# c0gent/hbbft

Hardware: AMD Instinct MI355X
Metric: verified BLS sig shares/sec (whole node) + combine latency, N=64 f=21 (higher is better)
Workload: dtype u32 limbs (Fp, 14x28-bit); 1 GPU; ThresholdSign share verification, BASELINE configs[1]; batch_per_gpu=65536, streams=2, documents_per_gpu=1024, n_nodes=64, f=21, pairing_impl=auto, parallelism=shard-by-batch x1

## Files before the change

hbbft_amd/csrc/ofp.hpp:

```cpp
#pragma once
#include "qfp.hpp"

namespace hbs {

HP_D int o_idx() { return (int)((threadIdx.x >> 1) & 3); }

HP_D int32_t o_swz4(int32_t v) { return __builtin_amdgcn_ds_swizzle(v, 0x101F); }
HP_D Fp o_swz4_fp(const Fp& a) {
  Fp r;
#pragma unroll
  for (int i = 0; i < NL; i++) r.l[i] = o_swz4(a.l[i]);
  return r;
}

HP_D Fp o_sel(int o, const Fp& a0, const Fp& a1, const Fp& a2, const Fp& a3) {
  const bool b0 = (o & 1) != 0, b1 = (o & 2) != 0;
  Fp r;
#pragma unroll
  for (int i = 0; i < NL; i++) {
    const int32_t lo = b0 ? a1.l[i] : a0.l[i];
    const int32_t hi = b0 ? a3.l[i] : a2.l[i];
    r.l[i] = b1 ? hi : lo;
  }
  return r;
// ... 128 lines not shown
  o.c1.c2 = fp_mul(f.c1.c2, fp_const(hb::FROB2_5_C0));
  return o;
}

HP_D HLine h_dbl_step_o(HJac& T) {
  Fp r[4];
  {
    const Fp x[4] = {T.x, T.y, T.z, fp_add(T.y, T.z)};
    h_sqr4(x, r);
  }
  const Fp A = r[0], B = r[1], ZZ = r[2], YZ = r[3];
  const Fp E = fp_lin(3, A, 0, A);
  {
    const Fp xb = fp_add(T.x, B);
    const Fp x[4] = {B, xb, E, E}, y[4] = {B, xb, E, T.x};
    h_mul4(x, y, r);
  }
  const Fp C = r[0], XB = r[1], F = r[2], EX = r[3];
  const Fp D = fp_lin(2, fp_sub(fp_sub(XB, A), C), 0, C);
  const Fp Z3 = fp_sub(fp_sub(YZ, B), ZZ);
  const Fp X3 = fp_sub(F, fp_add(D, D));
  {
    const Fp x[4] = {E, Z3, E, E}, y[4] = {ZZ, ZZ, fp_sub(D, X3), ZZ};
    h_mul4(x, y, r);
  }
  HLine l;
  l.c0 = fp_reduce(fp_sub(EX, fp_add(B, B)));
  l.c1 = fp_neg(r[0]);
  l.c4 = r[1];
  T.y = fp_reduce(fp_sub(r[2], fp_lin(8, C, 0, C)));
  T.x = fp_reduce(X3);
  T.z = fp_reduce(Z3);
  return l;
}

HP_D HLine h_add_step_o(HJac& T, const Fp& xQ, const Fp& yQ) {
  Fp r[4];
  {
    const Fp x[4] = {T.z, yQ, T.z, T.z}, y[4] = {T.z, T.z, T.z, T.z};
    h_mul4(x, y, r);
  }
  const Fp Z1Z1 = r[0], YZ = r[1];
  {
    const Fp x[4] = {xQ, YZ, xQ, xQ}, y[4] = {Z1Z1, Z1Z1, Z1Z1, Z1Z1};
    h_mul4(x, y, r);
  }
  const Fp H = fp_sub(r[0], T.x);
  const Fp rr = fp_sub(r[1], T.y);
  {
    const Fp x[4] = {H, rr, T.z, H}, y[4] = {H, rr, H, H};
    h_mul4(x, y, r);
  }
  const Fp HH = r[0], R2 = r[1], Z3 = r[2];
  {
    const Fp x[4] = {H, T.x, yQ, rr}, y[4] = {HH, HH, Z3, xQ};
    h_mul4(x, y, r);
  }
  const Fp HHH = r[0], V = r[1], YZ3 = r[2], RX = r[3];
  const Fp X3 = fp_sub(fp_sub(R2, HHH), fp_add(V, V));
  {
    const Fp x[4] = {rr, T.y, rr, rr}, y[4] = {fp_sub(V, X3), HHH, fp_sub(V, X3), fp_sub(V, X3)};
    h_mul4(x, y, r);
  }
  HLine l;
  l.c0 = fp_reduce(fp_sub(RX, YZ3));
  l.c1 = fp_neg(rr);
  l.c4 = Z3;
  T.x = fp_reduce(X3);
  T.y = fp_reduce(fp_sub(r[0], r[1]));
  T.z = Z3;
  return l;
}

struct LaneOcto {
  static constexpr int LANES = 8;
  static HP_D bool leader() { return (threadIdx.x & 7) == 0; }
  static HP_D bool value_writer() { return o_idx() == 0; }
  using Walk = HJac;
  template <bool W1, bool W2, int GEN>
  using Park = NoPark;
  static HP_D HLine dbl_step(HJac& T) { return h_dbl_step_o(T); }
  static HP_D HLine add_step(HJac& T, const Fp& xQ, const Fp& yQ) { return h_add_step_o(T, xQ, yQ); }

  static HP_D H6 mul6(const H6& a, const H6& b) { return h6_mul_o(a, b); }
  template <class A1, class B1>
  static HP_D void mul6x2(const H6& a0, const H6& b0, const A1& a1, const B1& b1, H6& r0, H6& r1) {
    h6_mul_pair_o(a0, b0, h6_of(a1), h6_of(b1), r0, r1);
  }
  static HP_D void mul6x2_12(const H6& a0, const H6& b0, const H6& a1, const Fp& c1, const Fp& c2, H6& r0, H6& r1) {
    h6_mul_pair_o(a0, b0, a1, {h_zero(), c1, c2}, r0, r1);
  }
  static HP_D void line_product(const Fp& a0, const Fp& a1, const Fp& a4, const Fp& b0, const Fp& b1, const Fp& b4,
                                H6& C0, Fp& c11, Fp& c12) {
    Fp r[4];
    {
      const Fp x[4] = {a0, a1, a4, fp_addl(a0, a4)}, y[4] = {b0, b1, b4, fp_add(b0, b4)};
      h_mul4(x, y, r);
    }
    const Fp a0b0 = r[0], a1b1 = r[1], a4b4 = r[2], t04 = r[3];
    {
      const Fp x[4] = {fp_addl(a1, a4), fp_addl(a0, a1), a0, a0}, y[4] = {fp_add(b1, b4), fp_add(b0, b1), b0, b0};
      h_mul4(x, y, r);
    }
    h_line_comb(a0b0, a1b1, a4b4, t04, r[0], r[1], C0, c11, c12);
  }
  static HP_D H12 cyclo_sqr(const H12& f) { return h12_cyclo_sqr_o(f); }
  static HP_D H12 frob1(const H12& f) { return h12_frob1_o(f); }
  static HP_D H12 frob2(const H12& f) { return h12_frob2_o(f); }

  template <bool G1, bool G2, bool WALK_FIRST, class RA, class RB, class ST>
  static HP_D void lines_at_p(const RA& raw_a, const RB& raw_b, const ST& A, const ST& B, bool neg2, HLine& la,
                              HLine& lb, const NoPark&) {
    const HLine ra = raw_a();
    const HLine rb = raw_b();
    Fp r[4];
    const Fp x[4] = {ra.c1, ra.c4, rb.c1, rb.c4};
    const Fp y[4] = {side_xP<G1>(A), side_yP<G1>(A, false), side_xP<G2>(B), side_yP<G2>(B, neg2)};
    fp_mul4(x, y, r);
    la.c0 = A.act ? ra.c0 : h_one();
    la.c1 = A.act ? r[0] : fp_zero();
    la.c4 = A.act ? r[1] : fp_zero();
    lb.c0 = B.act ? rb.c0 : h_one();
    lb.c1 = B.act ? r[2] : fp_zero();
    lb.c4 = B.act ? r[3] : fp_zero();
  }
};

}
```

hbbft_amd/csrc/pair_side.hpp:

```cpp
#pragma once
#include "launch.hpp"
#include "qfp.hpp"

namespace hbs {

constexpr int PAIR_STEPS = 68;
constexpr int PL_Q4 = 11;
constexpr int STASH_WORDS = 72;
static_assert(PARK_WORDS <= STASH_WORDS, "the Miller loop parks T and P in the stash (pfp.hpp PairPark)");

HP_D void stash_fp(uint32_t* __restrict__ s, const Fp& a) {
  const Fp r = fp_reduce(a);
  Fp rp = fp_addl(r, fp_const(P_L));
  fp_norm(rp);
  const Fp c = (r.l[NL - 1] < 0) ? rp : r;
#pragma unroll
  for (int w = 0; w < 12; w++) {
    const int bit = 32 * w, li = bit / 28, sh = bit % 28;
    uint64_t v = (uint64_t)(uint32_t)c.l[li] >> sh;
    if (li + 1 < NL) v |= (uint64_t)(uint32_t)c.l[li + 1] << (28 - sh);
    if (li + 2 < NL) v |= (uint64_t)(uint32_t)c.l[li + 2] << (56 - sh);
    s[w * 256] = (uint32_t)v;
  }
}
// ... 113 lines not shown

template <class G, bool WALK, bool DBL, int SIDE, class ST, class PK>
HP_D HLine side_raw(const PairSide& s, ST& st, int step, const PK& pk) {
  if constexpr (!WALK) {
    return line_load(s.lines + line_at(st.q * PAIR_STEPS + step));
  } else if constexpr (DBL) {
    return pk.template walk<SIDE>(st, [&](typename G::Walk& T) HP_L { return G::dbl_step(T); });
  } else {
    Fp xQ, yQ;
    side_q(s, st, xQ, yQ);
    return pk.template walk<SIDE>(st, [&](typename G::Walk& T) HP_L { return G::add_step(T, xQ, yQ); });
  }
}

struct PairArgs {
  int n;
  PairSide s1, s2;
  int flags;
  uint8_t* verdict;
  uint32_t* value_out;
};


template <class G, bool PLUS1>
HP_D H12 exp_abs_x_gs(const H12& base) {
  const uint64_t e = PLUS1 ? hb::X_ABS + 1 : hb::X_ABS;
  H12 r = base;
#pragma unroll 1
  for (int k = 62; k >= 0; k--) {
    r = G::cyclo_sqr(r);
    if ((e >> k) & 1) r = h12_mul<G>(r, base);
  }
  return r;
}
template <class G>
struct ExpGs {
  HP_D H12 x(const H12& f) { return h12_conj(exp_abs_x_gs<G, false>(f)); }
  HP_D H12 xm1(const H12& f) { return h12_conj(exp_abs_x_gs<G, true>(f)); }
};

template <class G, class Exp>
HP_D H12 final_exp(const H12& f, uint32_t* __restrict__ stash) {
  const H12 f1 = h12_mul<G>(h12_conj(f), h12_inv<G>(f));
  const H12 g = h12_mul<G>(G::frob2(f1), f1);
  stash12(stash, g);
  Exp ex;
  H12 a = ex.xm1(ex.xm1(g));
  const H12 b = h12_mul<G>(ex.x(a), G::frob1(a));
  {
    const H12 gs = unstash12(stash);
    const H12 w = h12_mul<G>(h12_mul<G>(G::frob2(b), h12_conj(b)), h12_mul<G>(G::cyclo_sqr(gs), gs));
    stash12(stash, w);
  }
  const H12 c = ex.x(ex.x(b));
  return h12_mul<G>(c, unstash12(stash));
}

template <class G, class Exp, bool W1, bool W2, int GEN>
HP_D void lane_verify(const PairArgs& a, uint32_t* stash) {
  const int i = (int)((blockIdx.x * 256u + threadIdx.x) / (unsigned)G::LANES);
  if (i >= a.n) return;
  constexpr bool G1 = GEN == 1, G2 = GEN == 2;
  const bool neg2 = (a.flags & 1) != 0;
  SideStateT<typename G::Walk> A, B;
  const bool ok1 = side_init<W1, G1>(a.s1, i, false, A);
  const bool ok2 = side_init<W2, G2>(a.s2, i, neg2, B);
  if (!ok1 || !ok2) {
    if (G::leader() && a.verdict) a.verdict[i] = 0;
    return;
  }
  const typename G::template Park<W1, W2, GEN> pk(stash + threadIdx.x);
  pk.init(A, B);
  constexpr bool WF = !W1 && W2;
  H12 f = h12_one();
  int step = 0;
#pragma unroll 1
  for (int b = 62; b >= 0; b--) {
    if (b != 62) f = h12_sqr<G>(f);
    {
      HLine la, lb;
      G::template lines_at_p<G1, G2, WF>([&]() HP_L { return side_raw<G, W1, true, 0>(a.s1, A, step, pk); },
                                         [&]() HP_L { return side_raw<G, W2, true, 1>(a.s2, B, step, pk); }, A, B, neg2,
                                         la, lb, pk);
      f = h12_mul_lines<G>(f, la.c0, la.c1, la.c4, lb.c0, lb.c1, lb.c4);
    }
    step++;
    if ((hb::X_ABS >> b) & 1) {
      HLine la, lb;
      G::template lines_at_p<G1, G2, WF>([&]() HP_L { return side_raw<G, W1, false, 0>(a.s1, A, step, pk); },
                                         [&]() HP_L { return side_raw<G, W2, false, 1>(a.s2, B, step, pk); }, A, B, neg2,
                                         la, lb, pk);
      f = h12_mul_lines<G>(f, la.c0, la.c1, la.c4, lb.c0, lb.c1, lb.c4);
      step++;
    }
  }
  if (a.flags & 2) f = h12_conj(f);
  const H12 e = final_exp<G, Exp>(f, stash + threadIdx.x);
  if (a.value_out && G::value_writer()) {
    uint32_t* o = a.value_out + (size_t)i * 144 + (lp_even() ? 0 : 12);
    fp_to_words(e.c0.c0, o + 0);
    fp_to_words(e.c0.c1, o + 24);
    fp_to_words(e.c0.c2, o + 48);
    fp_to_words(e.c1.c0, o + 72);
    fp_to_words(e.c1.c1, o + 96);
    fp_to_words(e.c1.c2, o + 120);
  }
  const bool one = h12_is_one(e);
  if (G::leader() && a.verdict) a.verdict[i] = one ? 1 : 0;
}

}

namespace hbl {

inline hbs::PairArgs pair_args(int n, const PairSideDesc& d1, const PairSideDesc& d2, int flags, uint8_t* verdict,
                               uint32_t* value_out) {
  hbs::PairArgs a;
  a.n = n;
  const PairSideDesc* d[2] = {&d1, &d2};
  hbs::PairSide* o[2] = {&a.s1, &a.s2};
  for (int k = 0; k < 2; k++) {
    o[k]->p = (const uint32_t*)d[k]->p;
    o[k]->q = (const uint32_t*)d[k]->q;
    o[k]->lines = (const int4*)d[k]->lines;
    o[k]->qinf = d[k]->qinf;
    o[k]->idx = d[k]->idx;
    o[k]->nq = (uint32_t)d[k]->nq;
  }
  a.flags = flags;
  a.verdict = verdict;
  a.value_out = value_out;
  return a;
}

inline int pair_gen_mode(const PairSideDesc& d1, const PairSideDesc& d2) {
  return (d1.p == nullptr) == (d2.p == nullptr) ? 0 : (d1.p == nullptr ? 1 : 2);
}

template <class K, int GEN>
hipError_t lane_launch(hipStream_t s, int n, const PairSideDesc& d1, const PairSideDesc& d2, int flags,
                       uint8_t* verdict, uint32_t* value_out) {
  const hbs::PairArgs a = pair_args(n, d1, d2, flags, verdict, value_out);
  const dim3 grid((unsigned)((K::LANES * (size_t)n + 255) / 256)), block(256);
  const size_t lds = (size_t)hbs::STASH_WORDS * 256 * 4;
  const bool w1 = d1.lines == nullptr, w2 = d2.lines == nullptr;
  if (w1 && w2)
    hipLaunchKernelGGL((K::template kernel<true, true, GEN>), grid, block, lds, s, a);
  else if (w1)
    hipLaunchKernelGGL((K::template kernel<true, false, GEN>), grid, block, lds, s, a);
  else if (w2)
    hipLaunchKernelGGL((K::template kernel<false, true, GEN>), grid, block, lds, s, a);
  else
    hipLaunchKernelGGL((K::template kernel<false, false, GEN>), grid, block, lds, s, a);
  return hipGetLastError();
}

}
```

hbbft_amd/csrc/pfp.hpp:

```cpp
#pragma once
#include "sfp.hpp"
#include "words.hpp"

#ifndef HP_INV_MODE
#define HP_INV_MODE 0
#endif

#define HP_D __device__ __forceinline__
#define HP_L __attribute__((always_inline))

namespace hbs {

constexpr int DPP_SWAP = 0xB1;
constexpr int DPP_EVEN = 0xA0;
constexpr int DPP_ODD = 0xF5;

HP_D bool lp_even() { return (threadIdx.x & 1) == 0; }
template <int CTRL>
HP_D int32_t dpp(int32_t v) {
  return __builtin_amdgcn_mov_dpp(v, CTRL, 0xF, 0xF, true);
}
template <int CTRL>
HP_D Fp dpp_fp(const Fp& a) {
  Fp r;
// ... 133 lines not shown
#pragma unroll
      for (int i = 0; i <= N; i++) row[i] = (t[i] >> 31) | (t[i + 1] << 1);
      const uint32_t fl = hb::words_abs<N + 1>(row);
      ks ^= fl;
      ss ^= (uint32_t)dpp<DPP_SWAP>((int32_t)fl);
#pragma unroll
      for (int i = 0; i < N; i++) {
        mine[i] = row[i];
        other[i] = (uint32_t)dpp<DPP_SWAP>((int32_t)row[i]);
      }
    }
    {
      uint32_t t[N + 2], w[N + 2];
      hb::words_mul_sm<N, true>(co, sm, ss, t);
#pragma unroll
      for (int i = 0; i < N + 2; i++) t[i] = (uint32_t)dpp<DPP_SWAP>((int32_t)t[i]);
      const uint32_t xe = 0u - (co[N] >> 31);
      const uint32_t k0 = km & ks;
      const uint64_t q = (uint64_t)(((k0 + (co[0] ^ ks) * km + t[0]) * minv) & 0x7fffffffu);
      uint64_t c = k0;
#pragma unroll
      for (int i = 0; i < N + 2; i++) {
        const uint32_t xi = (i <= N ? co[i] : xe) ^ ks;
        c += (uint64_t)xi * km;
        if (i < N) c += q * mod[i];
        c += t[i];
        w[i] = (uint32_t)c;
        c >>= 32;
      }
#pragma unroll
      for (int i = 0; i <= N; i++) co[i] = (w[i] >> 31) | (w[i + 1] << 1);
    }
  }
  const uint32_t mine_one = hb::words_is_one<N>(mine) ? 1u : 0u;
  const uint32_t part_one = (uint32_t)dpp<DPP_SWAP>((int32_t)mine_one);
  const bool one = (ev ? part_one : mine_one) != 0;
  uint32_t v[N + 1];
#pragma unroll
  for (int i = 0; i <= N; i++) {
    const uint32_t pv = (uint32_t)dpp<DPP_SWAP>((int32_t)co[i]);
    v[i] = ev ? pv : co[i];
  }
  hb::words_reduce_32m<N>(v, mod);
#pragma unroll
  for (int i = 0; i < N; i++) out[i] = one ? v[i] : 0u;
}

template <int MODE = 0>
HP_D Fp h_inv_vartime(const Fp& a) {
  const Fp s = fp_sqr(a);
  const Fp n = fp_add(s, dpp_fp<DPP_SWAP>(s));
  uint32_t w[12], p[12], r[12];
  fp_to_words(n, w);
  uint32_t nz = 0;
#pragma unroll
  for (int i = 0; i < 12; i++) nz |= w[i];
  if (nz == 0) return fp_zero();
#pragma unroll
  for (int i = 0; i < 12; i++) p[i] = hb::PM2_W[i];
  p[0] += 2;
  if ((MODE & INV_PAIR) != 0)
    lp_inv_uniform<12>(w, p, r);
  else
    hb::words_inv_vartime<12, MODE>(w, p, r);
  return h_conj(fp_mul(a, fp_from_words(r)));
}

template <int M, int K>
HP_D Fp fp_red_mk(const Fp& t, const Fp& a) {
  const int64_t top = (int64_t)t.l[NL - 1] * M + (int64_t)K * a.l[NL - 1];
  const int32_t q = (int32_t)((top * QINV) >> 32);
  Fp r;
  int64_t acc = 0;
#pragma unroll
  for (int i = 0; i < NL - 1; i++) {
    acc += (int64_t)t.l[i] * M + (int64_t)K * a.l[i] - (int64_t)q * (int32_t)P_L[i];
    r.l[i] = (int32_t)acc & MASK28;
    acc >>= 28;
  }
  r.l[NL - 1] = (int32_t)(acc + top - (int64_t)q * (int32_t)P_L[NL - 1]);
  return r;
}
HP_D Fp fp_red_l(const Fp& t) { return fp_red_mk<1, 0>(t, t); }
HP_D Fp h_add_xi_l(const Fp& s, const Fp& t) {
  const int32_t sm = lp_even() ? -1 : 0;
  const Fp pt = dpp_fp<DPP_SWAP>(t);
  Fp r;
#pragma unroll
  for (int i = 0; i < NL; i++) r.l[i] = s.l[i] + t.l[i] + ((pt.l[i] ^ sm) - sm);
  return r;
}
HP_D Fp fp_sub2l(const Fp& a, const Fp& b, const Fp& c) {
  Fp r;
#pragma unroll
  for (int i = 0; i < NL; i++) r.l[i] = a.l[i] - b.l[i] - c.l[i];
  return r;
}

HP_D Fp h_xi_l(const Fp& t) {
  const int32_t sm = lp_even() ? -1 : 0;
  const Fp pt = dpp_fp<DPP_SWAP>(t);
  Fp r;
#pragma unroll
  for (int i = 0; i < NL; i++) r.l[i] = t.l[i] + ((pt.l[i] ^ sm) - sm);
  return r;
}

struct H6 { Fp c0, c1, c2; };
struct H12 { H6 c0, c1; };

HP_D H6 h6_zero() { return {h_zero(), h_zero(), h_zero()}; }
HP_D H6 h6_one() { return {h_one(), h_zero(), h_zero()}; }
HP_D H6 h6_add(const H6& a, const H6& b) { return {fp_add(a.c0, b.c0), fp_add(a.c1, b.c1), fp_add(a.c2, b.c2)}; }
HP_D H6 h6_sub(const H6& a, const H6& b) { return {fp_sub(a.c0, b.c0), fp_sub(a.c1, b.c1), fp_sub(a.c2, b.c2)}; }
HP_D H6 h6_neg(const H6& a) { return {fp_neg(a.c0), fp_neg(a.c1), fp_neg(a.c2)}; }
HP_D H6 h6_red(const H6& a) { return {fp_reduce(a.c0), fp_reduce(a.c1), fp_reduce(a.c2)}; }
HP_D H6 h6_mul_v(const H6& a) { return {h_mul_xi(a.c2), a.c0, a.c1}; }

HP_D H6 h6_mul(const H6& a, const H6& b) {
  const Fp v1 = h_mul(a.c1, b.c1);
  const Fp v2 = h_mul(a.c2, b.c2);
  const Fp d0 = fp_sub2l(h_mul(fp_addl(a.c1, a.c2), fp_add(b.c1, b.c2)), v1, v2);
  const Fp v0 = h_mul(a.c0, b.c0);
  const Fp c0 = fp_red_l(h_add_xi_l(v0, d0));
  const Fp c1 = fp_red_l(h_add_xi_l(fp_sub2l(h_mul(fp_addl(a.c0, a.c1), fp_add(b.c0, b.c1)), v0, v1), v2));
  const Fp c2 = fp_red_l(fp_addl(fp_sub2l(h_mul(fp_addl(a.c0, a.c2), fp_add(b.c0, b.c2)), v0, v2), v1));
  return {c0, c1, c2};
}
HP_D H6 h6_inv(const H6& a) {
  const Fp c0 = fp_reduce(fp_sub(h_sqr(a.c0), h_mul_xi(h_mul(a.c1, a.c2))));
  const Fp c1 = fp_reduce(fp_sub(h_mul_xi(h_sqr(a.c2)), h_mul(a.c0, a.c1)));
  const Fp c2 = fp_reduce(fp_sub(h_sqr(a.c1), h_mul(a.c0, a.c2)));
  const Fp t = fp_reduce(fp_add(h_mul(a.c0, c0), h_mul_xi(fp_add(h_mul(a.c2, c1), h_mul(a.c1, c2)))));
  const Fp ti = fp_reduce(h_inv_vartime<HP_INV_MODE>(t));
  return {h_mul(c0, ti), h_mul(c1, ti), h_mul(c2, ti)};
}

HP_D H12 h12_one() { return {h6_one(), h6_zero()}; }
HP_D H12 h12_conj(const H12& a) { return {a.c0, h6_neg(a.c1)}; }
HP_D H12 h12_red(const H12& a) { return {h6_red(a.c0), h6_red(a.c1)}; }
HP_D H12 h12_kcomb(const H6& t0, const H6& t1, const H6& s) {
  return {{fp_red_l(h_add_xi_l(t0.c0, t1.c2)), fp_red_l(fp_addl(t0.c1, t1.c0)), fp_red_l(fp_addl(t0.c2, t1.c1))},
          {fp_red_l(fp_sub2l(s.c0, t0.c0, t1.c0)), fp_red_l(fp_sub2l(s.c1, t0.c1, t1.c1)),
           fp_red_l(fp_sub2l(s.c2, t0.c2, t1.c2))}};
}

HP_D H6 h6_mul_12(const H6& x, const Fp& b1, const Fp& b2) {
  const Fp u = h_mul(x.c1, b1);
  const Fp w = h_mul(x.c2, b2);
  const Fp c0 = fp_red_l(h_xi_l(fp_sub2l(h_mul(fp_addl(x.c1, x.c2), fp_add(b1, b2)), u, w)));
  const Fp c1 = fp_red_l(h_add_xi_l(h_mul(x.c0, b1), w));
  const Fp c2 = fp_red_l(fp_addl(h_mul(x.c0, b2), u));
  return {c0, c1, c2};
}

HP_D const H6& h6_of(const H6& a) { return a; }
template <class F>
HP_D auto h6_of(const F& f) -> decltype(f()) { return f(); }

template <class G>
HP_D H12 h12_mul(const H12& a, const H12& b) {
  H6 t0, t1;
  G::mul6x2(a.c0, b.c0, a.c1, b.c1, t0, t1);
  const H6 s = G::mul6(h6_add(a.c0, a.c1), h6_add(b.c0, b.c1));
  return h12_kcomb(t0, t1, s);
}
template <class G>
HP_D H12 h12_sqr(const H12& a) {
  H6 t, s;
  G::mul6x2(a.c0, a.c1, [&]() HP_L { return h6_add(a.c0, a.c1); },
            [&]() HP_L { return h6_red(h6_add(a.c0, h6_mul_v(a.c1))); }, t, s);
  return {{fp_red_l(h_add_xi_l(fp_subl(s.c0, t.c0), fp_subl(fp_zero(), t.c2))), fp_red_l(fp_sub2l(s.c1, t.c1, t.c0)),
           fp_red_l(fp_sub2l(s.c2, t.c2, t.c1))},
          {fp_red_l(fp_addl(t.c0, t.c0)), fp_red_l(fp_addl(t.c1, t.c1)), fp_red_l(fp_addl(t.c2, t.c2))}};
}
template <class G>
HP_D H12 h12_mul_lines(const H12& f, const Fp& a0, const Fp& a1, const Fp& a4, const Fp& b0, const Fp& b1,
                       const Fp& b4) {
  H6 C0, t0, t1;
  Fp c11, c12;
  G::line_product(a0, a1, a4, b0, b1, b4, C0, c11, c12);
  G::mul6x2_12(f.c0, C0, f.c1, c11, c12, t0, t1);
  const H6 s = G::mul6(h6_add(f.c0, f.c1), {C0.c0, fp_add(C0.c1, c11), fp_add(C0.c2, c12)});
  return h12_kcomb(t0, t1, s);
}
template <class G>
HP_D H12 h12_inv(const H12& a) {
  H6 s0, s1, r0, r1;
  G::mul6x2(a.c0, a.c0, a.c1, a.c1, s0, s1);
  const H6 t = h6_red(h6_sub(h6_red(s0), h6_red(h6_mul_v(h6_red(s1)))));
  const H6 ti = h6_red(h6_inv(t));
  G::mul6x2(a.c0, ti, a.c1, ti, r0, r1);
  return h12_red({r0, h6_neg(r1)});
}

#define HP_FROB1(K) h_const(hb::FROB1_##K##_C0, hb::FROB1_##K##_C1)
HP_D H12 h12_frob1(const H12& f) {
  H12 r;
  r.c0.c0 = h_conj(f.c0.c0);
  r.c1.c0 = h_mul(h_conj(f.c1.c0), HP_FROB1(1));
  r.c0.c1 = h_mul(h_conj(f.c0.c1), HP_FROB1(2));
  r.c1.c1 = h_mul(h_conj(f.c1.c1), HP_FROB1(3));
  r.c0.c2 = h_mul(h_conj(f.c0.c2), HP_FROB1(4));
  r.c1.c2 = h_mul(h_conj(f.c1.c2), HP_FROB1(5));
  return h12_red(r);
}
HP_D H12 h12_frob2(const H12& f) {
  H12 r;
  r.c0.c0 = f.c0.c0;
  r.c1.c0 = fp_mul(f.c1.c0, fp_const(hb::FROB2_1_C0));
  r.c0.c1 = fp_mul(f.c0.c1, fp_const(hb::FROB2_2_C0));
  r.c1.c1 = fp_mul(f.c1.c1, fp_const(hb::FROB2_3_C0));
  r.c0.c2 = fp_mul(f.c0.c2, fp_const(hb::FROB2_4_C0));
  r.c1.c2 = fp_mul(f.c1.c2, fp_const(hb::FROB2_5_C0));
  return r;
}

HP_D H12 h12_cyclo_sqr(const H12& f) {
  const Fp& a0 = f.c0.c0; const Fp& a2 = f.c0.c1; const Fp& a4 = f.c0.c2;
  const Fp& a1 = f.c1.c0; const Fp& a3 = f.c1.c1; const Fp& a5 = f.c1.c2;
  H12 r;
  {
    const Fp s0 = h_sqr(a0), s3 = h_sqr(a3), s03 = h_sqr(fp_add(a0, a3));
    r.c0.c0 = fp_red_mk<3, -2>(h_add_xi_l(s0, s3), a0);
    r.c1.c1 = fp_red_mk<3, 2>(fp_sub2l(s03, s0, s3), a3);
  }
  {
    const Fp s1 = h_sqr(a1), s4 = h_sqr(a4), s14 = h_sqr(fp_add(a1, a4));
    r.c0.c1 = fp_red_mk<3, -2>(h_add_xi_l(s1, s4), a2);
    r.c1.c2 = fp_red_mk<3, 2>(fp_sub2l(s14, s1, s4), a5);
  }
  {
    const Fp s2 = h_sqr(a2), s5 = h_sqr(a5), s25 = h_sqr(fp_add(a2, a5));
    r.c0.c2 = fp_red_mk<3, -2>(h_add_xi_l(s2, s5), a4);
    r.c1.c0 = fp_red_mk<3, 2>(h_add_xi_l(fp_zero(), fp_sub2l(s25, s2, s5)), a1);
  }
  return r;
}

struct HC { Fp a1, a2, a4, a5; };

HP_D HC hc_compress(const H12& f) { return {f.c1.c0, f.c0.c1, f.c0.c2, f.c1.c2}; }
HP_D HC hc_sqr(const HC& c) {
  HC r;
  {
    const Fp s1 = h_sqr(c.a1), s4 = h_sqr(c.a4), s14 = h_sqr(fp_add(c.a1, c.a4));
    r.a2 = fp_red_mk<3, -2>(h_add_xi_l(s1, s4), c.a2);
    r.a5 = fp_red_mk<3, 2>(fp_sub2l(s14, s1, s4), c.a5);
  }
  {
    const Fp s2 = h_sqr(c.a2), s5 = h_sqr(c.a5), s25 = h_sqr(fp_add(c.a2, c.a5));
    r.a4 = fp_red_mk<3, -2>(h_add_xi_l(s2, s5), c.a4);
    r.a1 = fp_red_mk<3, 2>(h_add_xi_l(fp_zero(), fp_sub2l(s25, s2, s5)), c.a1);
  }
  return r;
}
HP_D Fp hc_denom(const Fp& a1) { return fp_lin(4, a1, 0, a1); }
HP_D H12 hc_decompress(const HC& c, const Fp& di) {
  const Fp s5 = h_sqr(c.a5), s2 = h_sqr(c.a2);
  Fp t = h_xi_l(s5);
#pragma unroll
  for (int i = 0; i < NL; i++) t.l[i] += 3 * s2.l[i];
  const Fp a3 = h_mul(fp_red_mk<1, -2>(t, c.a4), di);
  const Fp u = fp_addl(fp_lin(2, h_sqr(a3), -3, h_mul(c.a4, c.a2)), h_mul(c.a1, c.a5));
  const Fp a0 = fp_red_l(h_add_xi_l(h_one(), u));
  return {{a0, c.a2, c.a4}, {c.a1, a3, c.a5}};
}
// ... 82 lines not shown

constexpr int PARK_WORDS = 72;
constexpr int park_fit(int used, bool need, int words) { return need && used + words <= PARK_WORDS ? used : -1; }
typedef volatile __attribute__((address_space(3))) uint32_t* ParkCol;

HP_D void park_put(ParkCol c, int slot, const Fp& a) {
#pragma unroll
  for (int i = 0; i < NL; i++) c[(slot + i) * 256] = (uint32_t)a.l[i];
}
HP_D Fp park_get(ParkCol c, int slot) {
  Fp r;
#pragma unroll
  for (int i = 0; i < NL; i++) r.l[i] = (int32_t)c[(slot + i) * 256];
  return r;
}

template <bool W1, bool W2, int GEN>
struct PairPark {
  static constexpr int TW = 3 * NL, PW = 2 * NL;
  static constexpr int T_B = park_fit(0, W2, TW);
  static constexpr int U1 = T_B < 0 ? 0 : TW;
  static constexpr int T_A = park_fit(U1, W1, TW);
  static constexpr int U2 = U1 + (T_A < 0 ? 0 : TW);
  static constexpr int P_A = park_fit(U2, GEN != 1, PW);
  static constexpr int U3 = U2 + (P_A < 0 ? 0 : PW);
  static constexpr int P_B = park_fit(U3, GEN != 2, PW);
  template <int SIDE>
  static constexpr int t_slot() { return SIDE == 0 ? T_A : T_B; }
  template <int SIDE>
  static constexpr int p_slot() { return SIDE == 0 ? P_A : P_B; }

  ParkCol col;
  HP_D explicit PairPark(uint32_t* c) : col((ParkCol)c) {}

  template <int SIDE>
  HP_D void put_T(const HProj& T) const {
    park_put(col, t_slot<SIDE>(), T.x);
    park_put(col, t_slot<SIDE>() + NL, T.y);
    park_put(col, t_slot<SIDE>() + 2 * NL, T.z);
  }
  template <int SIDE, class ST>
  HP_D void init_side(const ST& st) const {
    if constexpr (t_slot<SIDE>() >= 0) put_T<SIDE>(st.T);
    if constexpr (p_slot<SIDE>() >= 0) {
      park_put(col, p_slot<SIDE>(), st.xP);
      park_put(col, p_slot<SIDE>() + NL, st.yP);
    }
  }
  template <class ST>
  HP_D void init(const ST& A, const ST& B) const {
    init_side<0>(A);
    init_side<1>(B);
  }
  template <int SIDE, class ST, class F>
  HP_D HLine walk(ST& st, const F& f) const {
    if constexpr (t_slot<SIDE>() < 0) {
      return f(st.T);
    } else {
      HProj T;
      T.z = park_get(col, t_slot<SIDE>() + 2 * NL);
      T.y = park_get(col, t_slot<SIDE>() + NL);
      T.x = park_get(col, t_slot<SIDE>());
      const HLine l = f(T);
      put_T<SIDE>(T);
      return l;
    }
  }
  template <int SIDE, class ST>
  HP_D Fp xP(const ST& st) const {
    if constexpr (p_slot<SIDE>() < 0) return st.xP; else return park_get(col, p_slot<SIDE>());
  }
  template <int SIDE, class ST>
  HP_D Fp yP(const ST& st) const {
    if constexpr (p_slot<SIDE>() < 0) return st.yP; else return park_get(col, p_slot<SIDE>() + NL);
  }
};

#ifndef HP_PARK
#define HP_PARK 1
#endif
#ifndef HP_WALK_FIRST
#define HP_WALK_FIRST 1
#endif

struct LanePair {
  static constexpr int LANES = 2;
  static HP_D bool leader() { return lp_even(); }
  static HP_D bool value_writer() { return true; }
  using Walk = HProj;
  static HP_D HLine dbl_step(HProj& T) { return h_dbl_step_h(T); }
  static HP_D HLine add_step(HProj& T, const Fp& xQ, const Fp& yQ) { return h_add_step_h(T, xQ, yQ); }

  static HP_D H6 mul6(const H6& a, const H6& b) { return h6_mul(a, b); }
  template <class A1, class B1>
  static HP_D void mul6x2(const H6& a0, const H6& b0, const A1& a1, const B1& b1, H6& r0, H6& r1) {
    r0 = h6_mul(a0, b0);
    r1 = h6_mul(h6_of(a1), h6_of(b1));
  }
  static HP_D void mul6x2_12(const H6& a0, const H6& b0, const H6& a1, const Fp& c1, const Fp& c2, H6& r0, H6& r1) {
    r0 = h6_mul(a0, b0);
    r1 = h6_mul_12(a1, c1, c2);
  }
  static HP_D void line_product(const Fp& a0, const Fp& a1, const Fp& a4, const Fp& b0, const Fp& b1, const Fp& b4,
                                H6& C0, Fp& c11, Fp& c12) {
    const Fp a0b0 = h_mul(a0, b0);
    const Fp a1b1 = h_mul(a1, b1);
    const Fp a4b4 = h_mul(a4, b4);
    c11 = fp_red_l(fp_sub2l(h_mul(fp_addl(a0, a4), fp_add(b0, b4)), a0b0, a4b4));
    c12 = fp_red_l(fp_sub2l(h_mul(fp_addl(a1, a4), fp_add(b1, b4)), a1b1, a4b4));
    C0 = {fp_red_l(h_add_xi_l(a0b0, a4b4)), fp_red_l(fp_sub2l(h_mul(fp_addl(a0, a1), fp_add(b0, b1)), a0b0, a1b1)),
          a1b1};
  }
  static HP_D H12 cyclo_sqr(const H12& f) { return h12_cyclo_sqr(f); }
  static HP_D H12 frob1(const H12& f) { return h12_frob1(f); }
  static HP_D H12 frob2(const H12& f) { return h12_frob2(f); }

#if HP_PARK
  template <bool W1, bool W2, int GEN>
  using Park = PairPark<W1, W2, GEN>;
#else
  template <bool W1, bool W2, int GEN>
  using Park = NoPark;
#endif

  template <bool GEN, int SIDE, class ST, class PK>
  static HP_D HLine line_at_p(const HLine& l, const ST& st, bool negate, const PK& pk) {
    HLine e;
    e.c0 = st.act ? l.c0 : h_one();
    const Fp c1 = fp_mul(l.c1, GEN ? side_xP<true>(st) : pk.template xP<SIDE>(st));
    e.c1 = st.act ? c1 : fp_zero();
    const Fp c4 = fp_mul(l.c4, GEN ? side_yP<true>(st, negate) : pk.template yP<SIDE>(st));
    e.c4 = st.act ? c4 : fp_zero();
    return e;
  }
  template <bool G1, bool G2, bool WALK_FIRST, class RA, class RB, class ST, class PK>
  static HP_D void lines_at_p(const RA& raw_a, const RB& raw_b, const ST& A, const ST& B, bool neg2, HLine& la,
                              HLine& lb, const PK& pk) {
    if constexpr (WALK_FIRST && HP_WALK_FIRST) {
      lb = line_at_p<G2, 1>(raw_b(), B, neg2, pk);
      la = line_at_p<G1, 0>(raw_a(), A, false, pk);
    } else {
      la = line_at_p<G1, 0>(raw_a(), A, false, pk);
      lb = line_at_p<G2, 1>(raw_b(), B, neg2, pk);
    }
  }
};

HP_D void h_g2_load(const uint32_t* __restrict__ w, Fp& x, Fp& y) {
  const int o = lp_even() ? 0 : 12;
  x = fp_from_words(w + o);
  y = fp_from_words(w + 24 + o);
}
HP_D bool words_zero(const uint32_t* __restrict__ w, int n) {
  uint32_t o = 0;
  for (int k = 0; k < n; k++) o |= w[k];
  return o == 0;
}

}
```

hbbft_amd/csrc/qfp.hpp:

```cpp
#pragma once
#include "pfp.hpp"

namespace hbs {

constexpr int DPP_QSWAP = 0x4E;

HP_D bool q_hi() { return (threadIdx.x & 2) != 0; }

HP_D Fp q_sel(bool hi, const Fp& a, const Fp& b) {
  Fp r;
#pragma unroll
  for (int i = 0; i < NL; i++) r.l[i] = hi ? b.l[i] : a.l[i];
  return r;
}
HP_D H6 q_sel6(bool hi, const H6& a, const H6& b) { return {q_sel(hi, a.c0, b.c0), q_sel(hi, a.c1, b.c1), q_sel(hi, a.c2, b.c2)}; }

HP_D void q_join(bool hi, const Fp& mine, Fp& v0, Fp& v1) {
  const Fp o = dpp_fp<DPP_QSWAP>(mine);
  v0 = q_sel(hi, mine, o);
  v1 = q_sel(hi, o, mine);
}
HP_D void q_join6(bool hi, const H6& mine, H6& v0, H6& v1) {
  q_join(hi, mine.c0, v0.c0, v1.c0);
  q_join(hi, mine.c1, v0.c1, v1.c1);
// ... 48 lines not shown
  r.c0.c0 = fp_red_mk<3, -2>(h_add_xi_l(s0, s3), a0);
  r.c1.c1 = fp_red_mk<3, 2>(fp_sub2l(s03, s0, s3), a3);
  r.c0.c1 = fp_red_mk<3, -2>(h_add_xi_l(s1, s4), a2);
  r.c1.c2 = fp_red_mk<3, 2>(fp_sub2l(s14, s1, s4), a5);
  r.c0.c2 = fp_red_mk<3, -2>(h_add_xi_l(s2, s5), a4);
  r.c1.c0 = fp_red_mk<3, 2>(h_add_xi_l(fp_zero(), fp_sub2l(s25, s2, s5)), a1);
  return r;
}

HP_D H12 h12_frob1_q(const H12& f) {
  H12 r;
  r.c0.c0 = h_conj(f.c0.c0);
  h_mul2(h_conj(f.c1.c0), HP_FROB1(1), h_conj(f.c0.c1), HP_FROB1(2), r.c1.c0, r.c0.c1);
  h_mul2(h_conj(f.c1.c1), HP_FROB1(3), h_conj(f.c0.c2), HP_FROB1(4), r.c1.c1, r.c0.c2);
  r.c1.c2 = h_mul(h_conj(f.c1.c2), HP_FROB1(5));
  return h12_red(r);
}
HP_D H12 h12_frob2_q(const H12& f) {
  H12 r;
  r.c0.c0 = f.c0.c0;
  fp_mul2(f.c1.c0, fp_const(hb::FROB2_1_C0), f.c0.c1, fp_const(hb::FROB2_2_C0), r.c1.c0, r.c0.c1);
  fp_mul2(f.c1.c1, fp_const(hb::FROB2_3_C0), f.c0.c2, fp_const(hb::FROB2_4_C0), r.c1.c1, r.c0.c2);
  r.c1.c2 = fp_mul(f.c1.c2, fp_const(hb::FROB2_5_C0));
  return r;
}

HP_D HLine h_dbl_step_q(HJac& T) {
  Fp A, B, C, ZZ, XB, YZ, EX, EZ, C4, F;
  h_sqr2(T.x, T.y, A, B);
  h_sqr2(B, T.z, C, ZZ);
  h_sqr2(fp_add(T.x, B), fp_add(T.y, T.z), XB, YZ);
  const Fp D = fp_lin(2, fp_sub(fp_sub(XB, A), C), 0, C);
  const Fp E = fp_lin(3, A, 0, A);
  h_mul2(E, T.x, E, ZZ, EX, EZ);
  HLine l;
  l.c0 = fp_sub(EX, fp_add(B, B));
  l.c1 = fp_neg(EZ);
  const Fp Z3 = fp_sub(fp_sub(YZ, B), ZZ);
  h_mul2(Z3, ZZ, E, E, C4, F);
  l.c4 = C4;
  const Fp X3 = fp_sub(F, fp_add(D, D));
  T.y = fp_sub(h_mul(E, fp_sub(D, X3)), fp_lin(8, C, 0, C));
  T.x = X3;
  T.z = Z3;
  l.c0 = fp_reduce(l.c0);
  T.x = fp_reduce(T.x);
  T.y = fp_reduce(T.y);
  T.z = fp_reduce(T.z);
  return l;
}

HP_D HLine h_add_step_q(HJac& T, const Fp& xQ, const Fp& yQ) {
  Fp YZ, U2, S2, Z3, HH, R2, HHH, V, RV, YH, RX, YZ3;
  const Fp Z1Z1 = h_sqr(T.z);
  h_mul2(yQ, T.z, xQ, Z1Z1, YZ, U2);
  const Fp H = fp_sub(U2, T.x);
  h_mul2(YZ, Z1Z1, T.z, H, S2, Z3);
  const Fp r = fp_sub(S2, T.y);
  h_sqr2(H, r, HH, R2);
  h_mul2(H, HH, T.x, HH, HHH, V);
  const Fp X3 = fp_sub(fp_sub(R2, HHH), fp_add(V, V));
  h_mul2(r, fp_sub(V, X3), T.y, HHH, RV, YH);
  h_mul2(r, xQ, yQ, Z3, RX, YZ3);
  HLine l;
  l.c0 = fp_reduce(fp_sub(RX, YZ3));
  l.c1 = fp_neg(r);
  l.c4 = Z3;
  T.x = fp_reduce(X3);
  T.y = fp_reduce(fp_sub(RV, YH));
  T.z = Z3;
  return l;
}

struct LaneQuad {
  static constexpr int LANES = 4;
  static HP_D bool leader() { return (threadIdx.x & 3) == 0; }
  static HP_D bool value_writer() { return !q_hi(); }
  using Walk = HJac;
  template <bool W1, bool W2, int GEN>
  using Park = NoPark;
  static HP_D HLine dbl_step(HJac& T) { return h_dbl_step_q(T); }
  static HP_D HLine add_step(HJac& T, const Fp& xQ, const Fp& yQ) { return h_add_step_q(T, xQ, yQ); }

  static HP_D H6 mul6(const H6& a, const H6& b) { return h6_mul_q(a, b); }
  template <class A1, class B1>
  static HP_D void mul6x2(const H6& a0, const H6& b0, const A1& a1, const B1& b1, H6& r0, H6& r1) {
    h6_mul2(a0, b0, h6_of(a1), h6_of(b1), r0, r1);
  }
  static HP_D void mul6x2_12(const H6& a0, const H6& b0, const H6& a1, const Fp& c1, const Fp& c2, H6& r0, H6& r1) {
    h6_mul2(a0, b0, a1, {h_zero(), c1, c2}, r0, r1);
  }
  static HP_D void line_product(const Fp& a0, const Fp& a1, const Fp& a4, const Fp& b0, const Fp& b1, const Fp& b4,
                                H6& C0, Fp& c11, Fp& c12) {
    Fp a0b0, a1b1, a4b4, t04, t14, t01;
    h_mul2(a0, b0, a1, b1, a0b0, a1b1);
    h_mul2(a4, b4, fp_addl(a0, a4), fp_add(b0, b4), a4b4, t04);
    h_mul2(fp_addl(a1, a4), fp_add(b1, b4), fp_addl(a0, a1), fp_add(b0, b1), t14, t01);
    h_line_comb(a0b0, a1b1, a4b4, t04, t14, t01, C0, c11, c12);
  }
  static HP_D H12 cyclo_sqr(const H12& f) { return h12_cyclo_sqr_q(f); }
  static HP_D H12 frob1(const H12& f) { return h12_frob1_q(f); }
  static HP_D H12 frob2(const H12& f) { return h12_frob2_q(f); }

  template <bool GEN, class ST>
  static HP_D HLine line_at_p(const HLine& l, const ST& st, bool negate) {
    HLine e;
    e.c0 = st.act ? l.c0 : h_one();
    Fp c1, c4;
    fp_mul2(l.c1, side_xP<GEN>(st), l.c4, side_yP<GEN>(st, negate), c1, c4);
    e.c1 = st.act ? c1 : fp_zero();
    e.c4 = st.act ? c4 : fp_zero();
    return e;
  }
  template <bool G1, bool G2, bool WALK_FIRST, class RA, class RB, class ST>
  static HP_D void lines_at_p(const RA& raw_a, const RB& raw_b, const ST& A, const ST& B, bool neg2, HLine& la,
                              HLine& lb, const NoPark&) {
    la = line_at_p<G1>(raw_a(), A, false);
    lb = line_at_p<G2>(raw_b(), B, neg2);
  }
};

}
```

Baseline: 3.779 million shares/s.

## Use Toom-3 Fp6 multiplication scaled by 6 in Miller loop and skip first line multiply

```diff
diff --git a/hbbft_amd/csrc/ofp.hpp b/hbbft_amd/csrc/ofp.hpp
--- a/hbbft_amd/csrc/ofp.hpp
+++ b/hbbft_amd/csrc/ofp.hpp
@@ -234,6 +234,9 @@
   static HP_D HLine dbl_step(HJac& T) { return h_dbl_step_o(T); }
   static HP_D HLine add_step(HJac& T, const Fp& xQ, const Fp& yQ) { return h_add_step_o(T, xQ, yQ); }
 
+  static constexpr int MILLER_SCALE = 1;
+  template <bool W1, bool W2>
+  static constexpr bool first_line() { return false; }
   static HP_D H6 mul6(const H6& a, const H6& b) { return h6_mul_o(a, b); }
   template <class A1, class B1>
   static HP_D void mul6x2(const H6& a0, const H6& b0, const A1& a1, const B1& b1, H6& r0, H6& r1) {
diff --git a/hbbft_amd/csrc/pair_side.hpp b/hbbft_amd/csrc/pair_side.hpp
--- a/hbbft_amd/csrc/pair_side.hpp
+++ b/hbbft_amd/csrc/pair_side.hpp
@@ -219,7 +219,8 @@
       G::template lines_at_p<G1, G2, WF>([&]() HP_L { return side_raw<G, W1, true, 0>(a.s1, A, step, pk); },
                                          [&]() HP_L { return side_raw<G, W2, true, 1>(a.s2, B, step, pk); }, A, B, neg2,
                                          la, lb, pk);
-      f = h12_mul_lines<G>(f, la.c0, la.c1, la.c4, lb.c0, lb.c1, lb.c4);
+      constexpr bool FL = G::template first_line<W1, W2>();
+      f = h12_mul_lines<G>(f, la.c0, la.c1, la.c4, lb.c0, lb.c1, lb.c4, FL && b == 62);
     }
     step++;
     if ((hb::X_ABS >> b) & 1) {
diff --git a/hbbft_amd/csrc/pfp.hpp b/hbbft_amd/csrc/pfp.hpp
--- a/hbbft_amd/csrc/pfp.hpp
+++ b/hbbft_amd/csrc/pfp.hpp
@@ -239,6 +239,27 @@
   return r;
 }
 HP_D Fp fp_red_l(const Fp& t) { return fp_red_mk<1, 0>(t, t); }
+HP_D Fp fp_red_124(const Fp& a, const Fp& b, const Fp& c) {
+  const int32_t top = a.l[NL - 1] + 2 * b.l[NL - 1] + 4 * c.l[NL - 1];
+  const int32_t q = (int32_t)(((int64_t)top * QINV) >> 32);
+  Fp r;
+  int64_t acc = 0;
+#pragma unroll
+  for (int i = 0; i < NL - 1; i++) {
+    acc += (int64_t)(a.l[i] + 2 * b.l[i] + 4 * c.l[i]) - (int64_t)q * (int32_t)P_L[i];
+    r.l[i] = (int32_t)acc & MASK28;
+    acc >>= 28;
+  }
+  r.l[NL - 1] = (int32_t)(acc + top - (int64_t)q * (int32_t)P_L[NL - 1]);
+  return r;
+}
+HP_D Fp fp_lin3(const Fp& a, int k1, const Fp& b, int k2, const Fp& c) {
+  Fp r;
+#pragma unroll
+  for (int i = 0; i < NL; i++) r.l[i] = a.l[i] + k1 * b.l[i] + k2 * c.l[i];
+  fp_norm(r);
+  return r;
+}
 HP_D Fp h_add_xi_l(const Fp& s, const Fp& t) {
   const int32_t sm = lp_even() ? -1 : 0;
   const Fp pt = dpp_fp<DPP_SWAP>(t);
@@ -284,6 +305,34 @@
   const Fp c2 = fp_red_l(fp_addl(fp_sub2l(h_mul(fp_addl(a.c0, a.c2), fp_add(b.c0, b.c2)), v0, v2), v1));
   return {c0, c1, c2};
 }
+HP_D H6 h6_mul6(const H6& a, const H6& b) {
+  Fp c2, m, e, k, h;
+  {
+    const Fp sa = fp_add(a.c0, a.c2);
+    const Fp p1 = h_mul(fp_addl(sa, a.c1), fp_lin3(b.c0, 1, b.c1, 1, b.c2));
+    const Fp pm = h_mul(fp_subl(sa, a.c1), fp_lin3(b.c0, -1, b.c1, 1, b.c2));
+    const Fp p0 = h_mul(a.c0, b.c0);
+    const Fp pi = h_mul(a.c2, b.c2);
+    const Fp xpi = h_xi_l(pi);
+    Fp w;
+#pragma unroll
+    for (int i = 0; i < NL; i++) {
+      w.l[i] = p1.l[i] + pm.l[i] - 2 * p0.l[i] - 2 * pi.l[i];
+      m.l[i] = 3 * (p0.l[i] - p1.l[i]) - pm.l[i];
+      e.l[i] = p1.l[i] - pm.l[i];
+      k.l[i] = p0.l[i] - 2 * xpi.l[i];
+      h.l[i] = 2 * pi.l[i] + xpi.l[i];
+    }
+    c2 = fp_red_mk<3, 0>(w, w);
+  }
+  const Fp t = fp_addl(h_mul(fp_red_124(a.c0, a.c1, a.c2), fp_lin3(b.c0, 2, b.c1, 4, b.c2)), m);
+  const Fp c0 = fp_red_mk<1, 6>(h_xi_l(t), k);
+  Fp g;
+#pragma unroll
+  for (int i = 0; i < NL; i++) g.l[i] = 3 * e.l[i] - t.l[i];
+  const Fp c1 = fp_red_mk<1, 6>(g, h);
+  return {c0, c1, c2};
+}
 HP_D H6 h6_inv(const H6& a) {
   const Fp c0 = fp_reduce(fp_sub(h_sqr(a.c0), h_mul_xi(h_mul(a.c1, a.c2))));
   const Fp c1 = fp_reduce(fp_sub(h_mul_xi(h_sqr(a.c2)), h_mul(a.c0, a.c1)));
@@ -302,12 +351,16 @@
            fp_red_l(fp_sub2l(s.c2, t0.c2, t1.c2))}};
 }
 
+template <int S = 1>
 HP_D H6 h6_mul_12(const H6& x, const Fp& b1, const Fp& b2) {
   const Fp u = h_mul(x.c1, b1);
   const Fp w = h_mul(x.c2, b2);
-  const Fp c0 = fp_red_l(h_xi_l(fp_sub2l(h_mul(fp_addl(x.c1, x.c2), fp_add(b1, b2)), u, w)));
-  const Fp c1 = fp_red_l(h_add_xi_l(h_mul(x.c0, b1), w));
-  const Fp c2 = fp_red_l(fp_addl(h_mul(x.c0, b2), u));
+  const Fp d0 = h_xi_l(fp_sub2l(h_mul(fp_addl(x.c1, x.c2), fp_add(b1, b2)), u, w));
+  const Fp c0 = fp_red_mk<S, 0>(d0, d0);
+  const Fp d1 = h_add_xi_l(h_mul(x.c0, b1), w);
+  const Fp c1 = fp_red_mk<S, 0>(d1, d1);
+  const Fp d2 = fp_addl(h_mul(x.c0, b2), u);
+  const Fp c2 = fp_red_mk<S, 0>(d2, d2);
   return {c0, c1, c2};
 }
 
@@ -325,21 +378,32 @@
 template <class G>
 HP_D H12 h12_sqr(const H12& a) {
   H6 t, s;
-  G::mul6x2(a.c0, a.c1, [&]() HP_L { return h6_add(a.c0, a.c1); },
-            [&]() HP_L { return h6_red(h6_add(a.c0, h6_mul_v(a.c1))); }, t, s);
+  const auto a1 = [&]() HP_L { return h6_add(a.c0, a.c1); };
+  const auto b1 = [&]() HP_L { return h6_red(h6_add(a.c0, h6_mul_v(a.c1))); };
+  if constexpr (G::MILLER_SCALE == 1)
+    G::mul6x2(a.c0, a.c1, a1, b1, t, s);
+  else
+    G::mul6x2_s(a.c0, a.c1, a1, b1, t, s);
   return {{fp_red_l(h_add_xi_l(fp_subl(s.c0, t.c0), fp_subl(fp_zero(), t.c2))), fp_red_l(fp_sub2l(s.c1, t.c1, t.c0)),
            fp_red_l(fp_sub2l(s.c2, t.c2, t.c1))},
           {fp_red_l(fp_addl(t.c0, t.c0)), fp_red_l(fp_addl(t.c1, t.c1)), fp_red_l(fp_addl(t.c2, t.c2))}};
 }
 template <class G>
 HP_D H12 h12_mul_lines(const H12& f, const Fp& a0, const Fp& a1, const Fp& a4, const Fp& b0, const Fp& b1,
-                       const Fp& b4) {
+                       const Fp& b4, bool first = false) {
   H6 C0, t0, t1;
   Fp c11, c12;
   G::line_product(a0, a1, a4, b0, b1, b4, C0, c11, c12);
-  G::mul6x2_12(f.c0, C0, f.c1, c11, c12, t0, t1);
-  const H6 s = G::mul6(h6_add(f.c0, f.c1), {C0.c0, fp_add(C0.c1, c11), fp_add(C0.c2, c12)});
-  return h12_kcomb(t0, t1, s);
+  if (first) return {C0, {h_zero(), c11, c12}};
+  if constexpr (G::MILLER_SCALE == 1) {
+    G::mul6x2_12(f.c0, C0, f.c1, c11, c12, t0, t1);
+    const H6 s = G::mul6(h6_add(f.c0, f.c1), {C0.c0, fp_add(C0.c1, c11), fp_add(C0.c2, c12)});
+    return h12_kcomb(t0, t1, s);
+  } else {
+    G::mul6x2_12_s(f.c0, C0, f.c1, c11, c12, t0, t1);
+    const H6 s = G::mul6_s(h6_add(f.c0, f.c1), {C0.c0, fp_add(C0.c1, c11), fp_add(C0.c2, c12)});
+    return h12_kcomb(t0, t1, s);
+  }
 }
 template <class G>
 HP_D H12 h12_inv(const H12& a) {
@@ -588,6 +652,12 @@
 #ifndef HP_WALK_FIRST
 #define HP_WALK_FIRST 1
 #endif
+#ifndef HP_TOOM
+#define HP_TOOM 1
+#endif
+#ifndef HP_FIRST_LINE
+#define HP_FIRST_LINE 1
+#endif
 
 struct LanePair {
   static constexpr int LANES = 2;
@@ -606,6 +676,19 @@
   static HP_D void mul6x2_12(const H6& a0, const H6& b0, const H6& a1, const Fp& c1, const Fp& c2, H6& r0, H6& r1) {
     r0 = h6_mul(a0, b0);
     r1 = h6_mul_12(a1, c1, c2);
+  }
+  static constexpr int MILLER_SCALE = HP_TOOM ? 6 : 1;
+  template <bool W1, bool W2>
+  static constexpr bool first_line() { return HP_FIRST_LINE == 2 || (HP_FIRST_LINE == 1 && (W1 || W2)); }
+  static HP_D H6 mul6_s(const H6& a, const H6& b) { return h6_mul6(a, b); }
+  template <class A1, class B1>
+  static HP_D void mul6x2_s(const H6& a0, const H6& b0, const A1& a1, const B1& b1, H6& r0, H6& r1) {
+    r0 = h6_mul6(a0, b0);
+    r1 = h6_mul6(h6_of(a1), h6_of(b1));
+  }
+  static HP_D void mul6x2_12_s(const H6& a0, const H6& b0, const H6& a1, const Fp& c1, const Fp& c2, H6& r0, H6& r1) {
+    r0 = h6_mul6(a0, b0);
+    r1 = h6_mul_12<6>(a1, c1, c2);
   }
   static HP_D void line_product(const Fp& a0, const Fp& a1, const Fp& a4, const Fp& b0, const Fp& b1, const Fp& b4,
                                 H6& C0, Fp& c11, Fp& c12) {
diff --git a/hbbft_amd/csrc/qfp.hpp b/hbbft_amd/csrc/qfp.hpp
--- a/hbbft_amd/csrc/qfp.hpp
+++ b/hbbft_amd/csrc/qfp.hpp
@@ -154,6 +154,9 @@
   static HP_D HLine dbl_step(HJac& T) { return h_dbl_step_q(T); }
   static HP_D HLine add_step(HJac& T, const Fp& xQ, const Fp& yQ) { return h_add_step_q(T, xQ, yQ); }
 
+  static constexpr int MILLER_SCALE = 1;
+  template <bool W1, bool W2>
+  static constexpr bool first_line() { return false; }
   static HP_D H6 mul6(const H6& a, const H6& b) { return h6_mul_q(a, b); }
   template <class A1, class B1>
   static HP_D void mul6x2(const H6& a0, const H6& b0, const A1& a1, const B1& b1, H6& r0, H6& r1) {
```

Result: faster. 3.854 million shares/s (median of 6 runs) (+2.0%).
